# jmoraispk/DeepMIMO

Hardware: AMD Instinct MI355X
Metric: user-channels/sec (higher is better)
Workload: dtype f16x3-split MFMA, f32 accumulate

## Files before the change

deepmimo_amd/csrc/k2c_beam_power.hip:

```cpp
#include "k2_mfma_frag.h"
#include "dmx_tuning.h"
#include <stdlib.h>

namespace dmx {

static constexpr int BP_SLOT = 16 * 1024;
static constexpr int BP_BUFS = 2;

struct BeamPowArgs {
    int64_t user_begin;
    int m_rx, ue_mh, n_beams;
    int M;
    int K;
    const int32_t* sc;
    double inv_n;
    const float2* ftab;
    const int32_t* fexp;
    float* out;
    int32_t* best;
    int adaptive;
};

__host__ __device__ inline size_t beam_pow_lds_bytes(int M, int NW) {
    const size_t nblk = ((size_t)M + 32 * NW - 1) / (32 * NW);
    return (size_t)BP_BUFS * (NW / 4) * BP_SLOT + LPAD * (8 + 4 + 4) + 16 + nblk * NW * 32 * 4;
}

template <int NW>
__global__ __launch_bounds__(NW * 64, 4) void k2c_beam_power(WsView ws, BeamPowArgs a, int64_t user_count) {
    constexpr int BP_WAVES = NW, BP_CHUNK = NW / 4, MAX_ROWS = 32 * NW;
    extern __shared__ __attribute__((aligned(16))) unsigned char smem[];
    unsigned char* bbuf = smem;
    float* bbuf_f = reinterpret_cast<float*>(smem);
    float2* qtab = reinterpret_cast<float2*>(smem + (size_t)BP_BUFS * BP_CHUNK * BP_SLOT);
    float* crtab = reinterpret_cast<float*>(qtab + LPAD);
    float* citab = crtab + LPAD;
    float* misc = citab + LPAD;
    float* rs = misc + 4;
    const int tid = threadIdx.x, lane = tid & 63;
    const int wave = __builtin_amdgcn_readfirstlane(tid >> 6);
    const int col = lane & 31, hh = lane >> 5;
    const int B = a.n_beams, M = a.M, P = ws.P;
    const int nwide = (a.K + 31) >> 5;
    const int nblk = (M + MAX_ROWS - 1) / MAX_ROWS;

    for (int64_t ul = blockIdx.x; ul < user_count; ul += gridDim.x) {
        const int64_t u = a.user_begin + ul;
        int n_act = ws.n_keep[u];
        n_act = n_act < LPAD ? n_act : LPAD;
        if (n_act == 0) {
            for (int b = tid; b < B; b += BP_WAVES * 64) a.out[(size_t)ul * B + b] = 0.f;
            if (a.best && tid == 0) a.best[ul] = -1;
            continue;
        }
        const size_t rb = (size_t)u * P;
        if (wave == 0) {
            float m = 0.f;
            if (lane < n_act) m = fmaxf(fabsf(ws.c_re[rb + lane]), fabsf(ws.c_im[rb + lane]));
            for (int off = 32; off > 0; off >>= 1) m = fmaxf(m, __shfl_xor(m, off));
            const int l0w = ((n_act - 1) >> 3) << 3;
            float a2 = 0.f;
            if (lane < n_act) a2 = fmaf(ws.c_re[rb + lane], ws.c_re[rb + lane], ws.c_im[rb + lane] * ws.c_im[rb + lane]);
            float m2 = a2, mw2 = lane >= l0w ? a2 : 0.f;
            for (int off = 32; off > 0; off >>= 1) { m2 = fmaxf(m2, __shfl_xor(m2, off)); mw2 = fmaxf(mw2, __shfl_xor(mw2, off)); }
            if (lane == 0) misc[3] = (a.adaptive && l0w >= 8 && mw2 * 4194304.0f <= m2) ? 1.f : 0.f;
            int e;
            (void)frexpf(m, &e);
            const float gs = ldexpf(1.0f, 10 - e);
            if (lane < LPAD) {
                const bool ok = lane < n_act;
                const double q = ok ? (double)ws.dn[rb + lane] * a.inv_n : 0.0;
                const double qh = rint(q * 4096.0) * (1.0 / 4096.0);
                qtab[lane] = make_float2((float)qh, (float)(q - qh));
                crtab[lane] = ok ? ws.c_re[rb + lane] * gs : 0.f;
                citab[lane] = ok ? ws.c_im[rb + lane] * gs : 0.f;
            }
            const int ea = 6 - a.fexp[ul];
            if (lane == 0) { misc[0] = ldexpf(1.0f, e - 10 - ea); misc[1] = ldexpf(1.0f, ea); misc[2] = gs; }
        }
        __syncthreads();
        const float ascale = misc[1];
        const int nfull = ((n_act + 7) >> 3) - (misc[3] != 0.f ? 1 : 0);

        for (int blk = 0; blk < nblk; ++blk) {
            const int row0 = blk * MAX_ROWS;
            const int nrows = (M - row0) < MAX_ROWS ? (M - row0) : MAX_ROWS;
            const int ntiles = (nrows + 31) >> 5;
            const int ntp = ntiles <= 1 ? 1 : (ntiles <= 2 ? 2 : (ntiles <= 4 ? 4 : 8));
            const int tile = wave & (ntp - 1), grp = wave / ntp, ngrp = BP_WAVES / ntp;
            const bool active = tile < ntiles;
            h8 Ah[4], Al[4];
#pragma unroll
            for (int s = 0; s < 4; ++s) { Ah[s] = h8{0, 0, 0, 0, 0, 0, 0, 0}; Al[s] = Ah[s]; }
            if (active) {
                const int r = row0 + (tile << 5) + col;
                const bool pok = r < M;
                const int rx = pok ? r / B : 0, bm = pok ? r - rx * B : 0;
                const double yr = (double)(rx % a.ue_mh), zr = (double)(rx / a.ue_mh);
                const float2* frow = a.ftab + ((size_t)ul * B + bm) * P;
#pragma unroll
                for (int s = 0; s < 4; ++s) {
                    if (8 * s < n_act) {
#pragma unroll
                        for (int jj = 0; jj < 4; ++jj) {
                            const int pl = 8 * s + 4 * hh + jj;
                            h2 vh = {(_Float16)0.f, (_Float16)0.f}, vl = vh;
                            if (pok && pl < n_act) {
                                float sn, cs;
                                sincos_rev(frac_rev(yr * ws.rx_y[rb + pl] + zr * ws.rx_z[rb + pl]), sn, cs);
                                const float2 f = frow[pl];
                                split2_f16((cs * f.x - sn * f.y) * ascale, (cs * f.y + sn * f.x) * ascale, vh, vl, ws.neg_one);
                            }
                            Ah[s][2 * jj] = vh[0]; Ah[s][2 * jj + 1] = vh[1];
                            Al[s][2 * jj] = vl[0]; Al[s][2 * jj + 1] = vl[1];
                        }
                    }
                }
            }
            typedef float pv2 __attribute__((ext_vector_type(2)));
            pv2 rowsum[8];
#pragma unroll
            for (int i = 0; i < 8; ++i) rowsum[i] = pv2{0.f, 0.f};

            auto generate = [&](int c0, int buf) {
                const int wsi = c0 + (wave >> 2), st = wave & 3;
                const int kidx = (wsi << 5) + col;
                const bool kok = wsi < nwide && kidx < a.K;
                const int kki = kok ? a.sc[kidx] : 0;
                const float kl = (float)(kki & 4095), kf = (float)kki;
                h8* slot = reinterpret_cast<h8*>(bbuf + (size_t)(buf * BP_CHUNK + (wave >> 2)) * BP_SLOT);
                h8 rh = h8{0, 0, 0, 0, 0, 0, 0, 0}, rl = rh, ih = rh, il = rh;
                if (kok && 8 * st < n_act) {
#pragma unroll
                    for (int jj = 0; jj < 4; ++jj) {
                        const int pl = 8 * st + 4 * hh + jj;
                        const float2 q = qtab[pl];
                        const float p1 = q.x * kl;
                        float sn, cs;
                        sincos_rev(fmaf(q.y, kf, p1 - rintf(p1)), sn, cs);
                        const float cr = crtab[pl], ci = citab[pl];
                        h2 vh, vl;
                        split2_f16(cr * cs + ci * sn, ci * cs - cr * sn, vh, vl, ws.neg_one);
                        const unsigned hb = __builtin_bit_cast(unsigned, vh), lb = __builtin_bit_cast(unsigned, vl);
                        const h2 reh = __builtin_bit_cast(h2, hb ^ 0x80000000u), rel = __builtin_bit_cast(h2, lb ^ 0x80000000u);
                        const h2 imh = __builtin_bit_cast(h2, __builtin_amdgcn_alignbit(hb, hb, 16));
                        const h2 iml = __builtin_bit_cast(h2, __builtin_amdgcn_alignbit(lb, lb, 16));
                        rh[2 * jj] = reh[0]; rh[2 * jj + 1] = reh[1]; rl[2 * jj] = rel[0]; rl[2 * jj + 1] = rel[1];
                        ih[2 * jj] = imh[0]; ih[2 * jj + 1] = imh[1]; il[2 * jj] = iml[0]; il[2 * jj + 1] = iml[1];
                    }
                }
                slot[(4 * st + 0) * 64 + lane] = rh;
                slot[(4 * st + 1) * 64 + lane] = rl;
                slot[(4 * st + 2) * 64 + lane] = ih;
                slot[(4 * st + 3) * 64 + lane] = il;
            };
            __syncthreads();
            generate(0, 0);
            __syncthreads();
            int buf = 0;
            for (int c0 = 0; c0 < nwide; c0 += BP_CHUNK, buf ^= 1) {
                if (c0 + BP_CHUNK < nwide) generate(c0 + BP_CHUNK, buf ^ 1);
                if (active) {
                    for (int j = grp; j < BP_CHUNK && c0 + j < nwide; j += ngrp) {
                        const h8* slot = reinterpret_cast<const h8*>(bbuf + (size_t)(buf * BP_CHUNK + j) * BP_SLOT);
                        f16v are, aim;
#pragma unroll
                        for (int i = 0; i < 16; ++i) { are[i] = 0.f; aim[i] = 0.f; }
#pragma unroll
                        for (int s = 0; s < 4; ++s) {
                            if (8 * s < n_act) {
                                const h8 rh = slot[(4 * s + 0) * 64 + lane], rl = slot[(4 * s + 1) * 64 + lane];
                                const h8 ih = slot[(4 * s + 2) * 64 + lane], il = slot[(4 * s + 3) * 64 + lane];
                                are = __builtin_amdgcn_mfma_f32_32x32x16_f16(Ah[s], rh, are, 0, 0, 0);
                                aim = __builtin_amdgcn_mfma_f32_32x32x16_f16(Ah[s], ih, aim, 0, 0, 0);
                                if (s >= nfull) continue;
                                are = __builtin_amdgcn_mfma_f32_32x32x16_f16(Ah[s], rl, are, 0, 0, 0);
                                aim = __builtin_amdgcn_mfma_f32_32x32x16_f16(Ah[s], il, aim, 0, 0, 0);
                                are = __builtin_amdgcn_mfma_f32_32x32x16_f16(Al[s], rh, are, 0, 0, 0);
                                aim = __builtin_amdgcn_mfma_f32_32x32x16_f16(Al[s], ih, aim, 0, 0, 0);
                            }
                        }
                        DMX_MFMA_RESULT_GUARD2(are, aim);
#pragma unroll
                        for (int i = 0; i < 8; ++i) {
                            const pv2 re = {are[2 * i], are[2 * i + 1]}, im = {aim[2 * i], aim[2 * i + 1]};
                            const pv2 p = __builtin_elementwise_fma(re, re, im * im);
                            rowsum[i] += pv2{__builtin_amdgcn_sqrtf(p.x), __builtin_amdgcn_sqrtf(p.y)};
                        }
                    }
                }
                __syncthreads();
            }
            if (active) {
#pragma unroll
                for (int i = 0; i < 16; ++i) {
                    float v = (i & 1) ? rowsum[i >> 1].y : rowsum[i >> 1].x;
                    for (int off = 16; off > 0; off >>= 1) v += __shfl_xor(v, off);
                    if (col == 0) rs[((blk * BP_WAVES + wave) << 5) + (i & 3) + 8 * (i >> 2) + 4 * hh] = v;
                }
            }
        }
        __syncthreads();
        const float norm = misc[0] / ((float)a.m_rx * (float)a.K);
        for (int b = tid; b < B; b += BP_WAVES * 64) {
            float t = 0.f;
            for (int rx = 0; rx < a.m_rx; ++rx) {
                const int r = rx * B + b, blk = r / MAX_ROWS, w = r - blk * MAX_ROWS, tile = w >> 5;
                const int nrows = (M - blk * MAX_ROWS) < MAX_ROWS ? (M - blk * MAX_ROWS) : MAX_ROWS;
                const int ntiles = (nrows + 31) >> 5;
                const int ntp = ntiles <= 1 ? 1 : (ntiles <= 2 ? 2 : (ntiles <= 4 ? 4 : 8));
                for (int g = 0; g < BP_WAVES / ntp; ++g) t += rs[((blk * BP_WAVES + g * ntp + tile) << 5) + (w & 31)];
            }
            t *= norm;
            a.out[(size_t)ul * B + b] = t;
            bbuf_f[b] = t;
        }
        __syncthreads();
        if (a.best && tid == 0) {
            int arg = 0;
            float mx = bbuf_f[0];
            for (int b = 1; b < B; ++b) { if (bbuf_f[b] > mx) { mx = bbuf_f[b]; arg = b; } }
            a.best[ul] = arg;
        }
        __syncthreads();
    }
}

int launch_beam_power(const dmx_params& prm, const WsView& ws, int64_t user_begin, int64_t user_count,
                      const float2* codebook, int n_beams, void* beam_ws, float* out_amp, int32_t* out_best, hipStream_t stream) {
    if (user_count == 0 || n_beams == 0) return DMX_OK;
    BeamTabs t;
    int rc = launch_beam_project(prm, ws, user_begin, user_count, codebook, n_beams, beam_ws, stream, &t);
    if (rc) return rc;
    BeamPowArgs a;
    a.user_begin = user_begin;
    a.m_rx = prm.ue_shape[0] * prm.ue_shape[1];
    a.ue_mh = prm.ue_shape[0];
    a.n_beams = n_beams;
    a.M = a.m_rx * n_beams;
    a.K = prm.n_selected;
    a.sc = prm.selected_subcarriers;
    a.inv_n = 1.0 / (double)prm.n_subcarriers;
    a.ftab = t.ftab;
    a.fexp = t.fexp;
    a.out = out_amp;
    a.best = out_best;
    a.adaptive = (prm.flags & DMX_FLAG_ADAPTIVE_TERMS) ? 1 : 0;
    const int nw = tuning_int("DMX_BEAM_WAVES", 8) == 4 ? 4 : 8;
    const size_t smem = beam_pow_lds_bytes(a.M, nw);
    if (smem > 160 * 1024) { set_error("%d x %d (rx, beam) rows are too many for the beam-power kernel", a.m_rx, n_beams); return DMX_ERR_SHAPE; }
    const auto kernel = nw == 4 ? k2c_beam_power<4> : k2c_beam_power<8>;
    int64_t grid = resident_workgroups(kernel, nw * 64, smem);
    const int64_t g4 = user_count / 4;
    if (g4 > grid) grid = g4 < 4 * grid ? g4 : 4 * grid;
    if (grid > user_count) grid = user_count;
    return launch_dyn_lds(kernel, "k2c_beam_power", dim3((unsigned)grid), dim3(nw * 64), smem, smem, stream, ws, a, user_count);
}

}
```

Before: 6.265 million.

## Stage beam tables and subcarrier indices in LDS and pack short path tails

Each row block now stages the per-beam ftab rows into a swizzled LDS buffer, and the per-user rx_y/rx_z values go into LDS double tables. This replaces the scattered global loads made while building the A fragments. The subcarrier index list is cached in LDS when it fits. When the last group of 8 paths holds two or fewer entries, the hi/lo f16 split is packed into one MFMA K-slice so fewer MFMAs are needed. The per-user setup is merged into the first block's staging phase, which saves a barrier. In exchange the kernel uses more LDS, which can lower occupancy, and the index logic is more complex.

```diff
diff --git a/deepmimo_amd/csrc/k2c_beam_power.hip b/deepmimo_amd/csrc/k2c_beam_power.hip
--- a/deepmimo_amd/csrc/k2c_beam_power.hip
+++ b/deepmimo_amd/csrc/k2c_beam_power.hip
@@ -19,11 +19,13 @@
     float* out;
     int32_t* best;
     int adaptive;
+    int pack;
+    int sc_lds;
 };
 
 __host__ __device__ inline size_t beam_pow_lds_bytes(int M, int NW) {
     const size_t nblk = ((size_t)M + 32 * NW - 1) / (32 * NW);
-    return (size_t)BP_BUFS * (NW / 4) * BP_SLOT + LPAD * (8 + 4 + 4) + 16 + nblk * NW * 32 * 4;
+    return (size_t)BP_BUFS * (NW / 4) * BP_SLOT + LPAD * (8 + 4 + 4) + 16 + LPAD * (8 + 8) + nblk * NW * 32 * 4;
 }
 
 template <int NW>
@@ -36,13 +38,19 @@
     float* crtab = reinterpret_cast<float*>(qtab + LPAD);
     float* citab = crtab + LPAD;
     float* misc = citab + LPAD;
-    float* rs = misc + 4;
+    double* rytab = reinterpret_cast<double*>(misc + 4);
+    double* rztab = rytab + LPAD;
+    float* rs = reinterpret_cast<float*>(rztab + LPAD);
     const int tid = threadIdx.x, lane = tid & 63;
     const int wave = __builtin_amdgcn_readfirstlane(tid >> 6);
-    const int col = lane & 31, hh = lane >> 5;
     const int B = a.n_beams, M = a.M, P = ws.P;
     const int nwide = (a.K + 31) >> 5;
     const int nblk = (M + MAX_ROWS - 1) / MAX_ROWS;
+    int32_t* sctab = reinterpret_cast<int32_t*>(rs + (size_t)nblk * BP_WAVES * 32);
+    if (a.sc_lds) {
+#pragma unroll 1
+        for (int k = tid; k < a.K; k += BP_WAVES * 64) sctab[k] = a.sc[k];
+    }
 
     for (int64_t ul = blockIdx.x; ul < user_count; ul += gridDim.x) {
         const int64_t u = a.user_begin + ul;
@@ -54,65 +62,116 @@
             continue;
         }
         const size_t rb = (size_t)u * P;
-        if (wave == 0) {
-            float m = 0.f;
-            if (lane < n_act) m = fmaxf(fabsf(ws.c_re[rb + lane]), fabsf(ws.c_im[rb + lane]));
-            for (int off = 32; off > 0; off >>= 1) m = fmaxf(m, __shfl_xor(m, off));
-            const int l0w = ((n_act - 1) >> 3) << 3;
-            float a2 = 0.f;
-            if (lane < n_act) a2 = fmaf(ws.c_re[rb + lane], ws.c_re[rb + lane], ws.c_im[rb + lane] * ws.c_im[rb + lane]);
-            float m2 = a2, mw2 = lane >= l0w ? a2 : 0.f;
-            for (int off = 32; off > 0; off >>= 1) { m2 = fmaxf(m2, __shfl_xor(m2, off)); mw2 = fmaxf(mw2, __shfl_xor(mw2, off)); }
-            if (lane == 0) misc[3] = (a.adaptive && l0w >= 8 && mw2 * 4194304.0f <= m2) ? 1.f : 0.f;
-            int e;
-            (void)frexpf(m, &e);
-            const float gs = ldexpf(1.0f, 10 - e);
-            if (lane < LPAD) {
-                const bool ok = lane < n_act;
-                const double q = ok ? (double)ws.dn[rb + lane] * a.inv_n : 0.0;
-                const double qh = rint(q * 4096.0) * (1.0 / 4096.0);
-                qtab[lane] = make_float2((float)qh, (float)(q - qh));
-                crtab[lane] = ok ? ws.c_re[rb + lane] * gs : 0.f;
-                citab[lane] = ok ? ws.c_im[rb + lane] * gs : 0.f;
-            }
-            const int ea = 6 - a.fexp[ul];
-            if (lane == 0) { misc[0] = ldexpf(1.0f, e - 10 - ea); misc[1] = ldexpf(1.0f, ea); misc[2] = gs; }
-        }
-        __syncthreads();
-        const float ascale = misc[1];
-        const int nfull = ((n_act + 7) >> 3) - (misc[3] != 0.f ? 1 : 0);
-
+        const int l0w = ((n_act - 1) >> 3) << 3;
+        const bool tail2 = a.pack && n_act - l0w <= 2;
         for (int blk = 0; blk < nblk; ++blk) {
+            int lv = lane;
+            asm volatile("" : "+v"(lv));
+            const int col = lv & 31, hh = lv >> 5;
             const int row0 = blk * MAX_ROWS;
             const int nrows = (M - row0) < MAX_ROWS ? (M - row0) : MAX_ROWS;
             const int ntiles = (nrows + 31) >> 5;
             const int ntp = ntiles <= 1 ? 1 : (ntiles <= 2 ? 2 : (ntiles <= 4 ? 4 : 8));
             const int tile = wave & (ntp - 1), grp = wave / ntp, ngrp = BP_WAVES / ntp;
             const bool active = tile < ntiles;
+            float2* fst = reinterpret_cast<float2*>(bbuf);
+            const bool allb = nrows >= B;
+            const int nslot = allb ? B : nrows;
+            const float2* fuser = a.ftab + (size_t)ul * B * P + (col < P ? col : P - 1);
+            const int b0 = allb ? 0 : row0 % B;
+            auto stage_load = [&](int s0, float2 (&v)[4]) {
+#pragma unroll
+                for (int i = 0; i < 4; ++i) {
+                    const int slot = s0 + 2 * BP_WAVES * i < nslot ? s0 + 2 * BP_WAVES * i : nslot - 1;
+                    v[i] = fuser[(size_t)(b0 + slot < B ? b0 + slot : b0 + slot - B) * P];
+                }
+            };
+            auto stage_store = [&](int s0, const float2 (&v)[4]) {
+#pragma unroll
+                for (int i = 0; i < 4; ++i) {
+                    const int slot = s0 + 2 * BP_WAVES * i < nslot ? s0 + 2 * BP_WAVES * i : nslot - 1;
+                    fst[slot * 32 + (col ^ (slot & 31))] = v[i];
+                }
+            };
+            float2 fv[4];
+            stage_load(2 * wave + hh, fv);
+            if (blk == 0 && wave == 0) {
+                const int li = lv < P ? lv : P - 1;
+                const float cre = ws.c_re[rb + li], cim = ws.c_im[rb + li], dnv = ws.dn[rb + li];
+                const double ryv = ws.rx_y[rb + li], rzv = ws.rx_z[rb + li];
+                const int ea = 6 - a.fexp[ul];
+                const bool ok = lv < n_act;
+                float m = ok ? fmaxf(fabsf(cre), fabsf(cim)) : 0.f;
+                for (int off = 32; off > 0; off >>= 1) m = fmaxf(m, __shfl_xor(m, off));
+                const float a2 = ok ? fmaf(cre, cre, cim * cim) : 0.f;
+                float m2 = a2, mw2 = lv >= l0w ? a2 : 0.f;
+                for (int off = 32; off > 0; off >>= 1) { m2 = fmaxf(m2, __shfl_xor(m2, off)); mw2 = fmaxf(mw2, __shfl_xor(mw2, off)); }
+                const float weak = (a.adaptive && l0w >= 8 && mw2 * 4194304.0f <= m2) ? 1.f : 0.f;
+                if (lv == 0) misc[3] = weak != 0.f ? 1.f : (tail2 ? 2.f : 0.f);
+                int e;
+                (void)frexpf(m, &e);
+                const float gs = ldexpf(1.0f, 10 - e);
+                if (lv < LPAD) {
+                    const double q = ok ? (double)dnv * a.inv_n : 0.0;
+                    const double qh = rint(q * 4096.0) * (1.0 / 4096.0);
+                    qtab[lv] = make_float2((float)qh, (float)(q - qh));
+                    crtab[lv] = ok ? cre * gs : 0.f;
+                    citab[lv] = ok ? cim * gs : 0.f;
+                    rytab[lv] = ok ? ryv : 0.0;
+                    rztab[lv] = ok ? rzv : 0.0;
+                }
+                if (lv == 0) { misc[0] = ldexpf(1.0f, e - 10 - ea); misc[1] = ldexpf(1.0f, ea); misc[2] = gs; }
+            }
+            stage_store(2 * wave + hh, fv);
+            for (int s0 = 2 * wave + hh + 8 * BP_WAVES; s0 < nslot; s0 += 8 * BP_WAVES) {
+                stage_load(s0, fv);
+                stage_store(s0, fv);
+            }
+            __syncthreads();
+            const float ascale = misc[1];
+            const int mode = __builtin_amdgcn_readfirstlane((int)misc[3]);
+            const int nfull = ((n_act + 7) >> 3) - (mode != 0 ? 1 : 0);
             h8 Ah[4], Al[4];
 #pragma unroll
             for (int s = 0; s < 4; ++s) { Ah[s] = h8{0, 0, 0, 0, 0, 0, 0, 0}; Al[s] = Ah[s]; }
             if (active) {
                 const int r = row0 + (tile << 5) + col;
                 const bool pok = r < M;
-                const int rx = pok ? r / B : 0, bm = pok ? r - rx * B : 0;
+                const int rx = pok ? r / B : 0;
                 const double yr = (double)(rx % a.ue_mh), zr = (double)(rx / a.ue_mh);
-                const float2* frow = a.ftab + ((size_t)ul * B + bm) * P;
+                const int slot = pok ? (allb ? r - rx * B : r - row0) : 0;
+                const float2* fl = fst + slot * 32;
 #pragma unroll
                 for (int s = 0; s < 4; ++s) {
                     if (8 * s < n_act) {
+                        const bool tl = tail2 && 8 * s == l0w, pk = tl && mode == 2;
+                        const int ho = tl ? 0 : 4 * hh;
+                        const double* ry = rytab + ho;
+                        const double* rz = rztab + ho;
+                        const int sx = ho ^ (slot & 31);
+                        h2 vh[4], vl[4];
 #pragma unroll
                         for (int jj = 0; jj < 4; ++jj) {
-                            const int pl = 8 * s + 4 * hh + jj;
-                            h2 vh = {(_Float16)0.f, (_Float16)0.f}, vl = vh;
-                            if (pok && pl < n_act) {
-                                float sn, cs;
-                                sincos_rev(frac_rev(yr * ws.rx_y[rb + pl] + zr * ws.rx_z[rb + pl]), sn, cs);
-                                const float2 f = frow[pl];
-                                split2_f16((cs * f.x - sn * f.y) * ascale, (cs * f.y + sn * f.x) * ascale, vh, vl, ws.neg_one);
+                            vh[jj] = h2{(_Float16)0.f, (_Float16)0.f}; vl[jj] = vh[jj];
+                            if (tl && jj >= 2) continue;
+                            const int pl = 8 * s + jj + ho;
+                            float sn, cs;
+                            sincos_rev(frac_rev(yr * ry[8 * s + jj] + zr * rz[8 * s + jj]), sn, cs);
+                            const float2 f = fl[(8 * s + jj) ^ sx];
+                            h2 xh, xl;
+                            split2_f16((cs * f.x - sn * f.y) * ascale, (cs * f.y + sn * f.x) * ascale, xh, xl, ws.neg_one);
+                            if (pok && pl < n_act && (!tl || pk || hh == 0)) { vh[jj] = xh; vl[jj] = xl; }
+                        }
+                        if (pk) {
+                            const h2 z = {(_Float16)0.f, (_Float16)0.f};
+                            const h2 e0 = hh ? vl[0] : vh[0], e1 = hh ? vl[1] : vh[1], e2 = hh ? z : vh[0], e3 = hh ? z : vh[1];
+                            Ah[s] = h8{e0[0], e0[1], e1[0], e1[1], e2[0], e2[1], e3[0], e3[1]};
+                        } else {
+#pragma unroll
+                            for (int jj = 0; jj < 4; ++jj) {
+                                Ah[s][2 * jj] = vh[jj][0]; Ah[s][2 * jj + 1] = vh[jj][1];
+                                Al[s][2 * jj] = vl[jj][0]; Al[s][2 * jj + 1] = vl[jj][1];
                             }
-                            Ah[s][2 * jj] = vh[0]; Ah[s][2 * jj + 1] = vh[1];
-                            Al[s][2 * jj] = vl[0]; Al[s][2 * jj + 1] = vl[1];
                         }
                     }
                 }
@@ -126,33 +185,52 @@
                 const int wsi = c0 + (wave >> 2), st = wave & 3;
                 const int kidx = (wsi << 5) + col;
                 const bool kok = wsi < nwide && kidx < a.K;
-                const int kki = kok ? a.sc[kidx] : 0;
+                int kki = 0;
+                if (a.sc_lds) {
+                    kki = sctab[kok ? kidx : 0];
+                    asm volatile("" : "+v"(kki));
+                } else if (kok) {
+                    kki = a.sc[kidx];
+                }
+                kki = kok ? kki : 0;
                 const float kl = (float)(kki & 4095), kf = (float)kki;
                 h8* slot = reinterpret_cast<h8*>(bbuf + (size_t)(buf * BP_CHUNK + (wave >> 2)) * BP_SLOT);
                 h8 rh = h8{0, 0, 0, 0, 0, 0, 0, 0}, rl = rh, ih = rh, il = rh;
+                auto path = [&](int pl, unsigned& reh, unsigned& rel, unsigned& imh, unsigned& iml) {
+                    const float2 q = qtab[pl];
+                    const float p1 = q.x * kl;
+                    float sn, cs;
+                    sincos_rev(fmaf(q.y, kf, p1 - rintf(p1)), sn, cs);
+                    const float cr = crtab[pl], ci = citab[pl];
+                    h2 vh, vl;
+                    split2_f16(cr * cs + ci * sn, ci * cs - cr * sn, vh, vl, ws.neg_one);
+                    const unsigned hb = __builtin_bit_cast(unsigned, vh), lb = __builtin_bit_cast(unsigned, vl);
+                    reh = hb ^ 0x80000000u; rel = lb ^ 0x80000000u;
+                    imh = __builtin_amdgcn_alignbit(hb, hb, 16); iml = __builtin_amdgcn_alignbit(lb, lb, 16);
+                };
+                typedef unsigned u4v __attribute__((ext_vector_type(4)));
                 if (kok && 8 * st < n_act) {
-#pragma unroll
-                    for (int jj = 0; jj < 4; ++jj) {
-                        const int pl = 8 * st + 4 * hh + jj;
-                        const float2 q = qtab[pl];
-                        const float p1 = q.x * kl;
-                        float sn, cs;
-                        sincos_rev(fmaf(q.y, kf, p1 - rintf(p1)), sn, cs);
-                        const float cr = crtab[pl], ci = citab[pl];
-                        h2 vh, vl;
-                        split2_f16(cr * cs + ci * sn, ci * cs - cr * sn, vh, vl, ws.neg_one);
-                        const unsigned hb = __builtin_bit_cast(unsigned, vh), lb = __builtin_bit_cast(unsigned, vl);
-                        const h2 reh = __builtin_bit_cast(h2, hb ^ 0x80000000u), rel = __builtin_bit_cast(h2, lb ^ 0x80000000u);
-                        const h2 imh = __builtin_bit_cast(h2, __builtin_amdgcn_alignbit(hb, hb, 16));
-                        const h2 iml = __builtin_bit_cast(h2, __builtin_amdgcn_alignbit(lb, lb, 16));
-                        rh[2 * jj] = reh[0]; rh[2 * jj + 1] = reh[1]; rl[2 * jj] = rel[0]; rl[2 * jj + 1] = rel[1];
-                        ih[2 * jj] = imh[0]; ih[2 * jj + 1] = imh[1]; il[2 * jj] = iml[0]; il[2 * jj + 1] = iml[1];
+                    if (mode == 2 && 8 * st == l0w) {
+                        unsigned reh[2], rel[2], imh[2], iml[2];
+#pragma unroll
+                        for (int jj = 0; jj < 2; ++jj) path(8 * st + jj, reh[jj], rel[jj], imh[jj], iml[jj]);
+                        const unsigned keep = hh ? 0u : ~0u;
+                        rh = __builtin_bit_cast(h8, u4v{reh[0], reh[1], rel[0] & keep, rel[1] & keep});
+                        ih = __builtin_bit_cast(h8, u4v{imh[0], imh[1], iml[0] & keep, iml[1] & keep});
+                    } else {
+                        unsigned reh[4], rel[4], imh[4], iml[4];
+#pragma unroll
+                        for (int jj = 0; jj < 4; ++jj) path(8 * st + 4 * hh + jj, reh[jj], rel[jj], imh[jj], iml[jj]);
+                        rh = __builtin_bit_cast(h8, u4v{reh[0], reh[1], reh[2], reh[3]});
+                        rl = __builtin_bit_cast(h8, u4v{rel[0], rel[1], rel[2], rel[3]});
+                        ih = __builtin_bit_cast(h8, u4v{imh[0], imh[1], imh[2], imh[3]});
+                        il = __builtin_bit_cast(h8, u4v{iml[0], iml[1], iml[2], iml[3]});
                     }
                 }
-                slot[(4 * st + 0) * 64 + lane] = rh;
-                slot[(4 * st + 1) * 64 + lane] = rl;
-                slot[(4 * st + 2) * 64 + lane] = ih;
-                slot[(4 * st + 3) * 64 + lane] = il;
+                slot[(4 * st + 0) * 64 + lv] = rh;
+                slot[(4 * st + 1) * 64 + lv] = rl;
+                slot[(4 * st + 2) * 64 + lv] = ih;
+                slot[(4 * st + 3) * 64 + lv] = il;
             };
             __syncthreads();
             generate(0, 0);
@@ -169,8 +247,8 @@
 #pragma unroll
                         for (int s = 0; s < 4; ++s) {
                             if (8 * s < n_act) {
-                                const h8 rh = slot[(4 * s + 0) * 64 + lane], rl = slot[(4 * s + 1) * 64 + lane];
-                                const h8 ih = slot[(4 * s + 2) * 64 + lane], il = slot[(4 * s + 3) * 64 + lane];
+                                const h8 rh = slot[(4 * s + 0) * 64 + lv], rl = slot[(4 * s + 1) * 64 + lv];
+                                const h8 ih = slot[(4 * s + 2) * 64 + lv], il = slot[(4 * s + 3) * 64 + lv];
                                 are = __builtin_amdgcn_mfma_f32_32x32x16_f16(Ah[s], rh, are, 0, 0, 0);
                                 aim = __builtin_amdgcn_mfma_f32_32x32x16_f16(Ah[s], ih, aim, 0, 0, 0);
                                 if (s >= nfull) continue;
@@ -247,7 +325,10 @@
     a.best = out_best;
     a.adaptive = (prm.flags & DMX_FLAG_ADAPTIVE_TERMS) ? 1 : 0;
     const int nw = tuning_int("DMX_BEAM_WAVES", 8) == 4 ? 4 : 8;
-    const size_t smem = beam_pow_lds_bytes(a.M, nw);
+    a.pack = tuning_int("DMX_BEAM_PACK", 1) ? 1 : 0;
+    size_t smem = beam_pow_lds_bytes(a.M, nw);
+    a.sc_lds = smem + (size_t)a.K * 4 <= (size_t)MFMA_LDS_MAX * nw / 8 ? 1 : 0;
+    if (a.sc_lds) smem += (size_t)a.K * 4;
     if (smem > 160 * 1024) { set_error("%d x %d (rx, beam) rows are too many for the beam-power kernel", a.m_rx, n_beams); return DMX_ERR_SHAPE; }
     const auto kernel = nw == 4 ? k2c_beam_power<4> : k2c_beam_power<8>;
     int64_t grid = resident_workgroups(kernel, nw * 64, smem);
```

Measured after the change: 6.260 million, median of 4. Within noise of the previous version (-0.1%).

## Specialize beam-power block on path-slab count and pack short tail slab

Applied to the files above, without the earlier changes.

Moves the per-block beam power work into a function templated on the number of 8-path slabs and on whether the last slab is reduced. The kernel picks the instance with a wave-uniform switch. When the tail slab holds at most two paths, its hi and lo parts are packed into a single MFMA operand, so that slab needs two MFMAs instead of six and stores fewer LDS slots. This removes runtime slab guards, lets register arrays shrink to the needed size, and skips generation for unused slabs, at the cost of eight kernel instantiations and more code size.

```diff
diff --git a/deepmimo_amd/csrc/k2c_beam_power.hip b/deepmimo_amd/csrc/k2c_beam_power.hip
--- a/deepmimo_amd/csrc/k2c_beam_power.hip
+++ b/deepmimo_amd/csrc/k2c_beam_power.hip
@@ -26,6 +26,181 @@
     return (size_t)BP_BUFS * (NW / 4) * BP_SLOT + LPAD * (8 + 4 + 4) + 16 + nblk * NW * 32 * 4;
 }
 
+struct BeamBlk {
+    unsigned char* bbuf;
+    const float2* qtab;
+    const float* crtab;
+    const float* citab;
+    float* rs;
+    int64_t ul;
+    size_t rb;
+    int n_act, nwide;
+    float ascale;
+    bool pack;
+};
+
+template <int NW, int NS, bool ONE>
+__device__ __forceinline__ void beam_block(const WsView& ws, const BeamPowArgs& a, const BeamBlk& c, int blk, int wave, int lane) {
+    constexpr int BP_WAVES = NW, BP_CHUNK = NW / 4, MAX_ROWS = 32 * NW;
+    constexpr int NF = ONE ? NS - 1 : NS;
+    asm volatile("" : "+v"(lane));
+    const int col = lane & 31, hh = lane >> 5;
+    const int B = a.n_beams, M = a.M, P = ws.P;
+    const int n_act = c.n_act, nwide = c.nwide;
+    const bool pack = ONE && (NS == 1 || c.pack);
+    const int row0 = blk * MAX_ROWS;
+    const int nrows = (M - row0) < MAX_ROWS ? (M - row0) : MAX_ROWS;
+    const int ntiles = (nrows + 31) >> 5;
+    const int ntp = ntiles <= 1 ? 1 : (ntiles <= 2 ? 2 : (ntiles <= 4 ? 4 : 8));
+    const int tile = wave & (ntp - 1), grp = wave / ntp, ngrp = BP_WAVES / ntp;
+    const bool active = tile < ntiles;
+    h8 Ah[NS], Al[NF ? NF : 1];
+#pragma unroll
+    for (int s = 0; s < NS; ++s) Ah[s] = h8{0, 0, 0, 0, 0, 0, 0, 0};
+#pragma unroll
+    for (int s = 0; s < (NF ? NF : 1); ++s) Al[s] = h8{0, 0, 0, 0, 0, 0, 0, 0};
+    if (active) {
+        const int r = row0 + (tile << 5) + col;
+        const bool pok = r < M;
+        const int rx = pok ? r / B : 0, bm = pok ? r - rx * B : 0;
+        const double yr = (double)(rx % a.ue_mh), zr = (double)(rx / a.ue_mh);
+        const float2* frow = a.ftab + ((size_t)c.ul * B + bm) * P;
+        const float ascale = c.ascale;
+        auto entry = [&](int pl, h2& vh, h2& vl) {
+            vh = h2{(_Float16)0.f, (_Float16)0.f};
+            vl = vh;
+            if (pok && pl < n_act) {
+                float sn, cs;
+                sincos_rev(frac_rev(yr * ws.rx_y[c.rb + pl] + zr * ws.rx_z[c.rb + pl]), sn, cs);
+                const float2 f = frow[pl];
+                split2_f16((cs * f.x - sn * f.y) * ascale, (cs * f.y + sn * f.x) * ascale, vh, vl, ws.neg_one);
+            }
+        };
+#pragma unroll
+        for (int s = 0; s < NS; ++s) {
+            if (ONE && s == NS - 1 && pack) {
+                h2 vh[2], vl[2];
+#pragma unroll
+                for (int jj = 0; jj < 2; ++jj) entry(8 * s + jj, vh[jj], vl[jj]);
+                const h8 hi = {vh[0][0], vh[0][1], vh[1][0], vh[1][1], vh[0][0], vh[0][1], vh[1][0], vh[1][1]};
+                const h8 lo = {vl[0][0], vl[0][1], vl[1][0], vl[1][1], 0, 0, 0, 0};
+                Ah[s] = hh ? lo : hi;
+            } else {
+#pragma unroll
+                for (int jj = 0; jj < 4; ++jj) {
+                    h2 vh, vl;
+                    entry(8 * s + 4 * hh + jj, vh, vl);
+                    Ah[s][2 * jj] = vh[0]; Ah[s][2 * jj + 1] = vh[1];
+                    if (s < NF) { Al[s][2 * jj] = vl[0]; Al[s][2 * jj + 1] = vl[1]; }
+                }
+            }
+        }
+    }
+    typedef float pv2 __attribute__((ext_vector_type(2)));
+    pv2 rowsum[8];
+#pragma unroll
+    for (int i = 0; i < 8; ++i) rowsum[i] = pv2{0.f, 0.f};
+
+    auto generate = [&](int c0, int buf) {
+        const int wsi = c0 + (wave >> 2), st = wave & 3;
+        if (st >= NS) return;
+        const int kidx = (wsi << 5) + col;
+        const bool kok = wsi < nwide && kidx < a.K;
+        const int kki = kok ? a.sc[kidx] : 0;
+        const float kl = (float)(kki & 4095), kf = (float)kki;
+        h8* slot = reinterpret_cast<h8*>(c.bbuf + (size_t)(buf * BP_CHUNK + (wave >> 2)) * BP_SLOT);
+        const bool tail = ONE && st == NS - 1;
+        h8 rh = h8{0, 0, 0, 0, 0, 0, 0, 0}, rl = rh, ih = rh, il = rh;
+        auto phasor = [&](int pl, h2& reh, h2& rel, h2& imh, h2& iml) {
+            const float2 q = c.qtab[pl];
+            const float p1 = q.x * kl;
+            float sn, cs;
+            sincos_rev(fmaf(q.y, kf, p1 - rintf(p1)), sn, cs);
+            const float cr = c.crtab[pl], ci = c.citab[pl];
+            h2 vh, vl;
+            split2_f16(cr * cs + ci * sn, ci * cs - cr * sn, vh, vl, ws.neg_one);
+            const unsigned hb = __builtin_bit_cast(unsigned, vh), lb = __builtin_bit_cast(unsigned, vl);
+            reh = __builtin_bit_cast(h2, hb ^ 0x80000000u); rel = __builtin_bit_cast(h2, lb ^ 0x80000000u);
+            imh = __builtin_bit_cast(h2, __builtin_amdgcn_alignbit(hb, hb, 16));
+            iml = __builtin_bit_cast(h2, __builtin_amdgcn_alignbit(lb, lb, 16));
+        };
+        if (kok) {
+            if (tail && pack) {
+                h2 reh[2], rel[2], imh[2], iml[2];
+#pragma unroll
+                for (int jj = 0; jj < 2; ++jj) phasor(8 * st + jj, reh[jj], rel[jj], imh[jj], iml[jj]);
+                const h8 r0 = {reh[0][0], reh[0][1], reh[1][0], reh[1][1], rel[0][0], rel[0][1], rel[1][0], rel[1][1]};
+                const h8 r1 = {reh[0][0], reh[0][1], reh[1][0], reh[1][1], 0, 0, 0, 0};
+                const h8 i0 = {imh[0][0], imh[0][1], imh[1][0], imh[1][1], iml[0][0], iml[0][1], iml[1][0], iml[1][1]};
+                const h8 i1 = {imh[0][0], imh[0][1], imh[1][0], imh[1][1], 0, 0, 0, 0};
+                rh = hh ? r1 : r0;
+                ih = hh ? i1 : i0;
+            } else {
+#pragma unroll
+                for (int jj = 0; jj < 4; ++jj) {
+                    h2 reh, rel, imh, iml;
+                    phasor(8 * st + 4 * hh + jj, reh, rel, imh, iml);
+                    rh[2 * jj] = reh[0]; rh[2 * jj + 1] = reh[1]; rl[2 * jj] = rel[0]; rl[2 * jj + 1] = rel[1];
+                    ih[2 * jj] = imh[0]; ih[2 * jj + 1] = imh[1]; il[2 * jj] = iml[0]; il[2 * jj + 1] = iml[1];
+                }
+            }
+        }
+        slot[(4 * st + 0) * 64 + lane] = rh;
+        slot[(4 * st + 2) * 64 + lane] = ih;
+        if (!tail) {
+            slot[(4 * st + 1) * 64 + lane] = rl;
+            slot[(4 * st + 3) * 64 + lane] = il;
+        }
+    };
+    __syncthreads();
+    generate(0, 0);
+    __syncthreads();
+    int buf = 0;
+    for (int c0 = 0; c0 < nwide; c0 += BP_CHUNK, buf ^= 1) {
+        if (c0 + BP_CHUNK < nwide) generate(c0 + BP_CHUNK, buf ^ 1);
+        if (active) {
+            for (int j = grp; j < BP_CHUNK && c0 + j < nwide; j += ngrp) {
+                const h8* slot = reinterpret_cast<const h8*>(c.bbuf + (size_t)(buf * BP_CHUNK + j) * BP_SLOT);
+                f16v are, aim;
+#pragma unroll
+                for (int i = 0; i < 16; ++i) { are[i] = 0.f; aim[i] = 0.f; }
+#pragma unroll
+                for (int s = 0; s < NF; ++s) {
+                    const h8 rh = slot[(4 * s + 0) * 64 + lane], rl = slot[(4 * s + 1) * 64 + lane];
+                    const h8 ih = slot[(4 * s + 2) * 64 + lane], il = slot[(4 * s + 3) * 64 + lane];
+                    are = __builtin_amdgcn_mfma_f32_32x32x16_f16(Ah[s], rh, are, 0, 0, 0);
+                    aim = __builtin_amdgcn_mfma_f32_32x32x16_f16(Ah[s], ih, aim, 0, 0, 0);
+                    are = __builtin_amdgcn_mfma_f32_32x32x16_f16(Ah[s], rl, are, 0, 0, 0);
+                    aim = __builtin_amdgcn_mfma_f32_32x32x16_f16(Ah[s], il, aim, 0, 0, 0);
+                    are = __builtin_amdgcn_mfma_f32_32x32x16_f16(Al[s], rh, are, 0, 0, 0);
+                    aim = __builtin_amdgcn_mfma_f32_32x32x16_f16(Al[s], ih, aim, 0, 0, 0);
+                }
+                if (ONE) {
+                    const h8 rh = slot[(4 * (NS - 1) + 0) * 64 + lane], ih = slot[(4 * (NS - 1) + 2) * 64 + lane];
+                    are = __builtin_amdgcn_mfma_f32_32x32x16_f16(Ah[NS - 1], rh, are, 0, 0, 0);
+                    aim = __builtin_amdgcn_mfma_f32_32x32x16_f16(Ah[NS - 1], ih, aim, 0, 0, 0);
+                }
+                DMX_MFMA_RESULT_GUARD2(are, aim);
+#pragma unroll
+                for (int i = 0; i < 8; ++i) {
+                    const pv2 re = {are[2 * i], are[2 * i + 1]}, im = {aim[2 * i], aim[2 * i + 1]};
+                    const pv2 p = __builtin_elementwise_fma(re, re, im * im);
+                    rowsum[i] += pv2{__builtin_amdgcn_sqrtf(p.x), __builtin_amdgcn_sqrtf(p.y)};
+                }
+            }
+        }
+        __syncthreads();
+    }
+    if (active) {
+#pragma unroll
+        for (int i = 0; i < 16; ++i) {
+            float v = (i & 1) ? rowsum[i >> 1].y : rowsum[i >> 1].x;
+            for (int off = 16; off > 0; off >>= 1) v += __shfl_xor(v, off);
+            if (col == 0) c.rs[((blk * BP_WAVES + wave) << 5) + (i & 3) + 8 * (i >> 2) + 4 * hh] = v;
+        }
+    }
+}
+
 template <int NW>
 __global__ __launch_bounds__(NW * 64, 4) void k2c_beam_power(WsView ws, BeamPowArgs a, int64_t user_count) {
     constexpr int BP_WAVES = NW, BP_CHUNK = NW / 4, MAX_ROWS = 32 * NW;
@@ -39,7 +214,6 @@
     float* rs = misc + 4;
     const int tid = threadIdx.x, lane = tid & 63;
     const int wave = __builtin_amdgcn_readfirstlane(tid >> 6);
-    const int col = lane & 31, hh = lane >> 5;
     const int B = a.n_beams, M = a.M, P = ws.P;
     const int nwide = (a.K + 31) >> 5;
     const int nblk = (M + MAX_ROWS - 1) / MAX_ROWS;
@@ -55,149 +229,48 @@
         }
         const size_t rb = (size_t)u * P;
         if (wave == 0) {
+            int tl = lane;
+            asm volatile("" : "+v"(tl));
             float m = 0.f;
-            if (lane < n_act) m = fmaxf(fabsf(ws.c_re[rb + lane]), fabsf(ws.c_im[rb + lane]));
+            if (tl < n_act) m = fmaxf(fabsf(ws.c_re[rb + tl]), fabsf(ws.c_im[rb + tl]));
             for (int off = 32; off > 0; off >>= 1) m = fmaxf(m, __shfl_xor(m, off));
             const int l0w = ((n_act - 1) >> 3) << 3;
             float a2 = 0.f;
-            if (lane < n_act) a2 = fmaf(ws.c_re[rb + lane], ws.c_re[rb + lane], ws.c_im[rb + lane] * ws.c_im[rb + lane]);
-            float m2 = a2, mw2 = lane >= l0w ? a2 : 0.f;
+            if (tl < n_act) a2 = fmaf(ws.c_re[rb + tl], ws.c_re[rb + tl], ws.c_im[rb + tl] * ws.c_im[rb + tl]);
+            float m2 = a2, mw2 = tl >= l0w ? a2 : 0.f;
             for (int off = 32; off > 0; off >>= 1) { m2 = fmaxf(m2, __shfl_xor(m2, off)); mw2 = fmaxf(mw2, __shfl_xor(mw2, off)); }
-            if (lane == 0) misc[3] = (a.adaptive && l0w >= 8 && mw2 * 4194304.0f <= m2) ? 1.f : 0.f;
+            if (tl == 0) misc[3] = (a.adaptive && l0w >= 8 && mw2 * 4194304.0f <= m2) ? 1.f : 0.f;
             int e;
             (void)frexpf(m, &e);
             const float gs = ldexpf(1.0f, 10 - e);
-            if (lane < LPAD) {
-                const bool ok = lane < n_act;
-                const double q = ok ? (double)ws.dn[rb + lane] * a.inv_n : 0.0;
+            if (tl < LPAD) {
+                const bool ok = tl < n_act;
+                const double q = ok ? (double)ws.dn[rb + tl] * a.inv_n : 0.0;
                 const double qh = rint(q * 4096.0) * (1.0 / 4096.0);
-                qtab[lane] = make_float2((float)qh, (float)(q - qh));
-                crtab[lane] = ok ? ws.c_re[rb + lane] * gs : 0.f;
-                citab[lane] = ok ? ws.c_im[rb + lane] * gs : 0.f;
+                qtab[tl] = make_float2((float)qh, (float)(q - qh));
+                crtab[tl] = ok ? ws.c_re[rb + tl] * gs : 0.f;
+                citab[tl] = ok ? ws.c_im[rb + tl] * gs : 0.f;
             }
             const int ea = 6 - a.fexp[ul];
-            if (lane == 0) { misc[0] = ldexpf(1.0f, e - 10 - ea); misc[1] = ldexpf(1.0f, ea); misc[2] = gs; }
-        }
-        __syncthreads();
-        const float ascale = misc[1];
-        const int nfull = ((n_act + 7) >> 3) - (misc[3] != 0.f ? 1 : 0);
+            if (tl == 0) { misc[0] = ldexpf(1.0f, e - 10 - ea); misc[1] = ldexpf(1.0f, ea); misc[2] = gs; }
+        }
+        __syncthreads();
+        const int l0w = ((n_act - 1) >> 3) << 3;
+        const bool weak = misc[3] != 0.f;
+        const bool pack = !weak && n_act - l0w <= 2;
+        const int kind = __builtin_amdgcn_readfirstlane(((n_act + 7) >> 3) + ((weak || pack) ? 4 : 0));
+        const BeamBlk c{bbuf, qtab, crtab, citab, rs, ul, rb, n_act, nwide, misc[1], pack};
 
         for (int blk = 0; blk < nblk; ++blk) {
-            const int row0 = blk * MAX_ROWS;
-            const int nrows = (M - row0) < MAX_ROWS ? (M - row0) : MAX_ROWS;
-            const int ntiles = (nrows + 31) >> 5;
-            const int ntp = ntiles <= 1 ? 1 : (ntiles <= 2 ? 2 : (ntiles <= 4 ? 4 : 8));
-            const int tile = wave & (ntp - 1), grp = wave / ntp, ngrp = BP_WAVES / ntp;
-            const bool active = tile < ntiles;
-            h8 Ah[4], Al[4];
-#pragma unroll
-            for (int s = 0; s < 4; ++s) { Ah[s] = h8{0, 0, 0, 0, 0, 0, 0, 0}; Al[s] = Ah[s]; }
-            if (active) {
-                const int r = row0 + (tile << 5) + col;
-                const bool pok = r < M;
-                const int rx = pok ? r / B : 0, bm = pok ? r - rx * B : 0;
-                const double yr = (double)(rx % a.ue_mh), zr = (double)(rx / a.ue_mh);
-                const float2* frow = a.ftab + ((size_t)ul * B + bm) * P;
-#pragma unroll
-                for (int s = 0; s < 4; ++s) {
-                    if (8 * s < n_act) {
-#pragma unroll
-                        for (int jj = 0; jj < 4; ++jj) {
-                            const int pl = 8 * s + 4 * hh + jj;
-                            h2 vh = {(_Float16)0.f, (_Float16)0.f}, vl = vh;
-                            if (pok && pl < n_act) {
-                                float sn, cs;
-                                sincos_rev(frac_rev(yr * ws.rx_y[rb + pl] + zr * ws.rx_z[rb + pl]), sn, cs);
-                                const float2 f = frow[pl];
-                                split2_f16((cs * f.x - sn * f.y) * ascale, (cs * f.y + sn * f.x) * ascale, vh, vl, ws.neg_one);
-                            }
-                            Ah[s][2 * jj] = vh[0]; Ah[s][2 * jj + 1] = vh[1];
-                            Al[s][2 * jj] = vl[0]; Al[s][2 * jj + 1] = vl[1];
-                        }
-                    }
-                }
-            }
-            typedef float pv2 __attribute__((ext_vector_type(2)));
-            pv2 rowsum[8];
-#pragma unroll
-            for (int i = 0; i < 8; ++i) rowsum[i] = pv2{0.f, 0.f};
-
-            auto generate = [&](int c0, int buf) {
-                const int wsi = c0 + (wave >> 2), st = wave & 3;
-                const int kidx = (wsi << 5) + col;
-                const bool kok = wsi < nwide && kidx < a.K;
-                const int kki = kok ? a.sc[kidx] : 0;
-                const float kl = (float)(kki & 4095), kf = (float)kki;
-                h8* slot = reinterpret_cast<h8*>(bbuf + (size_t)(buf * BP_CHUNK + (wave >> 2)) * BP_SLOT);
-                h8 rh = h8{0, 0, 0, 0, 0, 0, 0, 0}, rl = rh, ih = rh, il = rh;
-                if (kok && 8 * st < n_act) {
-#pragma unroll
-                    for (int jj = 0; jj < 4; ++jj) {
-                        const int pl = 8 * st + 4 * hh + jj;
-                        const float2 q = qtab[pl];
-                        const float p1 = q.x * kl;
-                        float sn, cs;
-                        sincos_rev(fmaf(q.y, kf, p1 - rintf(p1)), sn, cs);
-                        const float cr = crtab[pl], ci = citab[pl];
-                        h2 vh, vl;
-                        split2_f16(cr * cs + ci * sn, ci * cs - cr * sn, vh, vl, ws.neg_one);
-                        const unsigned hb = __builtin_bit_cast(unsigned, vh), lb = __builtin_bit_cast(unsigned, vl);
-                        const h2 reh = __builtin_bit_cast(h2, hb ^ 0x80000000u), rel = __builtin_bit_cast(h2, lb ^ 0x80000000u);
-                        const h2 imh = __builtin_bit_cast(h2, __builtin_amdgcn_alignbit(hb, hb, 16));
-                        const h2 iml = __builtin_bit_cast(h2, __builtin_amdgcn_alignbit(lb, lb, 16));
-                        rh[2 * jj] = reh[0]; rh[2 * jj + 1] = reh[1]; rl[2 * jj] = rel[0]; rl[2 * jj + 1] = rel[1];
-                        ih[2 * jj] = imh[0]; ih[2 * jj + 1] = imh[1]; il[2 * jj] = iml[0]; il[2 * jj + 1] = iml[1];
-                    }
-                }
-                slot[(4 * st + 0) * 64 + lane] = rh;
-                slot[(4 * st + 1) * 64 + lane] = rl;
-                slot[(4 * st + 2) * 64 + lane] = ih;
-                slot[(4 * st + 3) * 64 + lane] = il;
-            };
-            __syncthreads();
-            generate(0, 0);
-            __syncthreads();
-            int buf = 0;
-            for (int c0 = 0; c0 < nwide; c0 += BP_CHUNK, buf ^= 1) {
-                if (c0 + BP_CHUNK < nwide) generate(c0 + BP_CHUNK, buf ^ 1);
-                if (active) {
-                    for (int j = grp; j < BP_CHUNK && c0 + j < nwide; j += ngrp) {
-                        const h8* slot = reinterpret_cast<const h8*>(bbuf + (size_t)(buf * BP_CHUNK + j) * BP_SLOT);
-                        f16v are, aim;
-#pragma unroll
-                        for (int i = 0; i < 16; ++i) { are[i] = 0.f; aim[i] = 0.f; }
-#pragma unroll
-                        for (int s = 0; s < 4; ++s) {
-                            if (8 * s < n_act) {
-                                const h8 rh = slot[(4 * s + 0) * 64 + lane], rl = slot[(4 * s + 1) * 64 + lane];
-                                const h8 ih = slot[(4 * s + 2) * 64 + lane], il = slot[(4 * s + 3) * 64 + lane];
-                                are = __builtin_amdgcn_mfma_f32_32x32x16_f16(Ah[s], rh, are, 0, 0, 0);
-                                aim = __builtin_amdgcn_mfma_f32_32x32x16_f16(Ah[s], ih, aim, 0, 0, 0);
-                                if (s >= nfull) continue;
-                                are = __builtin_amdgcn_mfma_f32_32x32x16_f16(Ah[s], rl, are, 0, 0, 0);
-                                aim = __builtin_amdgcn_mfma_f32_32x32x16_f16(Ah[s], il, aim, 0, 0, 0);
-                                are = __builtin_amdgcn_mfma_f32_32x32x16_f16(Al[s], rh, are, 0, 0, 0);
-                                aim = __builtin_amdgcn_mfma_f32_32x32x16_f16(Al[s], ih, aim, 0, 0, 0);
-                            }
-                        }
-                        DMX_MFMA_RESULT_GUARD2(are, aim);
-#pragma unroll
-                        for (int i = 0; i < 8; ++i) {
-                            const pv2 re = {are[2 * i], are[2 * i + 1]}, im = {aim[2 * i], aim[2 * i + 1]};
-                            const pv2 p = __builtin_elementwise_fma(re, re, im * im);
-                            rowsum[i] += pv2{__builtin_amdgcn_sqrtf(p.x), __builtin_amdgcn_sqrtf(p.y)};
-                        }
-                    }
-                }
-                __syncthreads();
-            }
-            if (active) {
-#pragma unroll
-                for (int i = 0; i < 16; ++i) {
-                    float v = (i & 1) ? rowsum[i >> 1].y : rowsum[i >> 1].x;
-                    for (int off = 16; off > 0; off >>= 1) v += __shfl_xor(v, off);
-                    if (col == 0) rs[((blk * BP_WAVES + wave) << 5) + (i & 3) + 8 * (i >> 2) + 4 * hh] = v;
-                }
+            switch (kind) {
+                case 1: beam_block<NW, 1, false>(ws, a, c, blk, wave, lane); break;
+                case 2: beam_block<NW, 2, false>(ws, a, c, blk, wave, lane); break;
+                case 3: beam_block<NW, 3, false>(ws, a, c, blk, wave, lane); break;
+                case 4: beam_block<NW, 4, false>(ws, a, c, blk, wave, lane); break;
+                case 5: beam_block<NW, 1, true>(ws, a, c, blk, wave, lane); break;
+                case 6: beam_block<NW, 2, true>(ws, a, c, blk, wave, lane); break;
+                case 7: beam_block<NW, 3, true>(ws, a, c, blk, wave, lane); break;
+                default: beam_block<NW, 4, true>(ws, a, c, blk, wave, lane); break;
             }
         }
         __syncthreads();
```

Result: no change. 6.278 million before, 6.266 million after, median of 2 (-0.2%).
